# RookieJunChen/FullSubNet-plus

Hardware: AMD Instinct MI355X
Metric: STFT frames/sec (257-bin, 2 s clips), FullSubNet+ forward (higher is better)
Workload: dtype f32

## Files before the change

fullsubnet_plus_amd/_lib.py:

```python
import ctypes
import os

from . import _build

c_i32, c_i64, c_f32p, c_vp = ctypes.c_int32, ctypes.c_int64, ctypes.POINTER(ctypes.c_float), ctypes.c_void_p


class FsnpConfig(ctypes.Structure):
    _fields_ = [
        ("num_freqs", c_i32), ("look_ahead", c_i32), ("sb_num_neighbors", c_i32), ("fb_num_neighbors", c_i32),
        ("tcn_hidden", c_i32), ("num_tcn_blocks", c_i32), ("sb_hidden", c_i32), ("output_size", c_i32),
        ("norm_type", c_i32), ("fb_act", c_i32), ("sb_act", c_i32), ("kersize", c_i32 * 3),
        ("num_groups_in_drop_band", c_i32), ("attention", c_i32), ("model", c_i32), ("sequence_model", c_i32),
        ("subband_num", c_i32),
    ]


NORM_TYPES = {"offline_laplace_norm": 0, "cumulative_laplace_norm": 1, "offline_gaussian_norm": 2,
              "cumulative_layer_norm": 3}
ACTIVATIONS = {None: 0, False: 0, "": 0, "ReLU": 1, "ReLU6": 2, "Tanh": 3}
ATTENTION = {"TSSE": 0, "SE": 1, "ECA": 2, "CBAM": 3}
SEQUENCE_MODELS = {"LSTM": 0, "GRU": 1, "TCN": 2}
MODE_FULL, MODE_PARITY = 0, 1
NUM_COSTS = 27
# ... 31 lines not shown
    "fsnp_get_costs": (c_i32, [c_vp, ctypes.POINTER(ctypes.c_double * NUM_COSTS), ctypes.POINTER(c_i32), ctypes.POINTER(c_i32)]),
    "fsnp_debug_plan_rows": (c_i32, [c_i32, c_i32, c_i32, c_i32, c_i32, ctypes.c_double, ctypes.POINTER(c_i32), c_i32]),
    "fsnp_measure_costs": (c_i32, [c_vp, ctypes.POINTER(ctypes.c_double * NUM_COSTS)]),
    "fsnp_debug_set_costs": (c_i32, [c_vp, ctypes.POINTER(ctypes.c_double), c_i32]),
    "fsnp_debug_plan_rows2": (c_i32, [c_i32, c_i32, c_i32, c_i32, c_i32, ctypes.c_double, c_i32, ctypes.POINTER(ctypes.c_double),
                              ctypes.POINTER(c_i32), c_i32]),
    "fsnp_debug_coop_side_by_side": (c_i32, [ctypes.POINTER(c_i32 * 8), c_i32, c_i32, ctypes.POINTER(c_i32 * 8), c_i32, c_i32, c_i32]),
    "fsnp_debug_fullsubnet_pairing": (c_i32, [c_i32, c_i32, c_i32, ctypes.POINTER(ctypes.c_double), ctypes.POINTER(c_i32), c_i32]),
    "fsnp_debug_pipeline_pairing": (c_i32, [c_vp, c_i32, ctypes.POINTER(c_i32), c_i32]),
    "fsnp_debug_coop_chain_stats": (c_i32, [c_vp, ctypes.POINTER(c_i64 * 2), c_i32]),
    "fsnp_debug_fullband_launch": (c_i32, [c_vp, c_i32, ctypes.POINTER(c_i32 * 4)]),
    "fsnp_forward_flops": (ctypes.c_double, [c_vp, c_i32, c_i32, c_i32]),
    "fsnp_lstm_flops": (ctypes.c_double, [c_vp, c_i64, c_i32]),
    "fsnp_debug_lstm_profile": (c_i32, [c_vp, c_vp, c_vp, c_i32, c_i32, c_vp, c_i64]),
    "fsnp_debug_pp_profile": (c_i32, [c_vp, c_vp, c_vp, c_i32, c_i32, c_i32, c_vp, c_i64]),
    "fsnp_set_precision": (c_i32, [c_vp, c_i32]),
    "fsnp_check_errors": (c_i32, [c_vp]),
    "fsnp_poll_errors": (c_i32, [c_vp]),
    "fsnp_set_pipeline": (c_i32, [c_vp, c_i32]),
    "fsnp_flush": (c_i32, [c_vp, c_vp]),
    "fsnp_watch_weights": (c_i32, [c_vp, ctypes.POINTER(c_vp), ctypes.POINTER(c_i64), c_i32, c_i32, c_vp]),
    "fsnp_set_verify": (c_i32, [c_vp, c_i32]),
    "fsnp_set_verify_sample": (c_i32, [c_vp, c_i32]),
    "fsnp_verify_count": (c_i64, [c_vp]),
    "fsnp_debug_verify_sample_stats": (c_i32, [c_vp, ctypes.POINTER(c_i64 * 3)]),
    "fsnp_debug_corrupt_exchange": (c_i32, [c_vp, c_i32]),
    "fsnp_abi_version": (c_i32, []),
    "fsnp_config_size": (c_i32, []),
    "fsnp_debug_set_lstm_coop": (c_i32, [c_vp, c_i32]),
    "fsnp_debug_set_gemm_dma": (c_i32, [c_vp, c_i32]),
    "fsnp_debug_inject_error": (c_i32, [c_vp]),
    "fsnp_debug_set_chaos": (c_i32, [c_vp, c_i32]),
    "fsnp_debug_set_lstm_waves": (c_i32, [c_vp, c_i32]),
    "fsnp_debug_set_num_cus": (c_i32, [c_vp, c_i32]),
    "fsnp_debug_lstm_pack": (c_i32, [c_i32, c_i32, c_i32, c_i32, c_vp, c_vp, c_vp, c_vp, c_vp, c_i64]),
    "fsnp_debug_lstm_coop_pack": (c_i32, [c_i32, c_i32, c_i32, c_i32, c_vp, c_vp, c_vp, c_vp, c_vp, c_i64]),
    "fsnp_debug_lstm_coopw_pack": (c_i32, [c_i32, c_i32, c_i32, c_vp, c_vp, c_vp, c_vp, c_vp, c_i64]),
    "fsnp_debug_lstm_hpw_pack": (c_i32, [c_i32, c_i32, c_i32, c_vp, c_vp, c_vp, c_vp, c_vp, c_i64]),
    "fsnp_debug_lstm_fbv_pack": (c_i32, [c_i32, c_i32, c_vp, c_vp, c_vp, c_vp, c_vp, c_i64]),
    "fsnp_debug_box_probe": (c_i32, [ctypes.c_double, ctypes.POINTER(ctypes.c_double * BOX_PROBE_VALUES), c_vp]),
    "fsnp_debug_launch_clock": (c_i32, [c_vp, ctypes.POINTER(ctypes.c_double * 7)]),
    "fsnp_last_error": (ctypes.c_char_p, []),
    "fsnp_version": (ctypes.c_char_p, []),
}

LENGTHS_SYMBOLS = {
    "fsnp_forward_lengths": (c_i32, [c_vp, c_vp, c_vp, c_vp, ctypes.POINTER(c_i64 * 3 * 3), ctypes.POINTER(c_i32), c_vp, c_i32, c_i32,
                                     c_vp]),
    "fsnp_forward_complex_lengths": (c_i32, [c_vp, c_vp, ctypes.POINTER(c_i64 * 3), ctypes.POINTER(c_i32), c_vp, c_i32, c_i32, c_vp]),
    "fsnp_enhance_wave_lengths": (c_i32, [c_vp, c_vp, c_i64, c_vp, c_i64, ctypes.POINTER(c_i32), c_i32, c_i32, c_vp]),
    "fsnp_apply_cirm_lengths": (c_i32, [c_vp, c_vp, ctypes.POINTER(c_i64 * 3), c_vp, ctypes.POINTER(c_i64 * 3), ctypes.POINTER(c_i32),
                                        c_i32, c_i32, c_i32, c_vp]),
}

STREAM_SYMBOLS = {
    "fsnp_stream_create": (c_i32, [c_vp, c_i32, c_i32, ctypes.POINTER(c_vp)]),
    "fsnp_stream_destroy": (None, [c_vp]),
    "fsnp_stream_push": (c_i32, [c_vp, c_vp, ctypes.POINTER(c_i64 * 3), ctypes.POINTER(c_i32), c_vp, c_i32, c_vp]),
    "fsnp_stream_reset": (c_i32, [c_vp, ctypes.POINTER(c_i32), c_i32, c_vp]),
    "fsnp_stream_state_bytes": (c_i64, [c_vp]),
    "fsnp_stream_get_state": (c_i32, [c_vp, c_i32, c_vp, c_vp]),
    "fsnp_stream_set_state": (c_i32, [c_vp, c_i32, c_vp, c_vp]),
    "fsnp_stream_frames": (c_i32, [c_vp, c_i32, ctypes.POINTER(c_i64)]),
}

ABI_VERSION = 13
# ... 46 lines not shown
```

fullsubnet_plus_amd/csrc/fsnp_common.h:

```cpp
#pragma once
#include <hip/hip_runtime.h>
#include <math.h>
#include <stdint.h>

#include "../../include/fsnp.h"
#include "../../include/fsnp_debug.h"

namespace fsnp {

struct Dims {
    int B;
    int T;
    int Tp;
    int F;
    int FP;
    int CH;
    int H;
    int NSB;
    int NIN;
    int LA;
    const int* lens = nullptr;
    const int* tpb = nullptr;
};

// ... 135 lines not shown
struct RowDesc { int b, f, out_off, valid; };
constexpr int kGnStride = 16;

void launch_subband_stats(const Dims& d, int norm_type, const SubbandBuffers& buf, const RowDesc* rows,
                          int num_slots, hipStream_t s);
struct SbGatherArgs {
    const float* att_mag; int fb_rel, fb_branch_stride;
    const RowDesc* rows; const NormMD* md_utt; const NormMD* md_row;
    float* x; int xstride;
    int num_slots, Tp, FP, F, NSBN, NFBN, NIN;
};
void launch_sb_gather(const SbGatherArgs& a, hipStream_t s);
void launch_sb_scatter(const float* y, int ystride, const RowDesc* rows, float* out, long out_stride_o, int num_slots,
                       int Tp, int LA, int out_channels, hipStream_t s);

struct LstmWeights {
    const float* wpack;
    const float* wpack12;
    const float* wpack_bf[2];
    int ih_bf16;
    const float* wpack_coop[4];
    const float* wpack_coopn;
    const float* wpack16;
    const float* wpack16_bf;
    const float* wpack_gru;
    const float* wpack_hp;
    const float* wpack_hpw;
    int hp_wave;
    const float* wpack_fbv;
    const float* wpack_coopw;
    const float* wgen;
    int gru;
    int waves;
    const float* bias;
    const float* wfc;
    const float* bfc;
    int H, NIN, KX, OUT;
};
struct LstmArgs {
    const float* att_mag;
    const float* fb;
    int fb_rel;
    int fb_branch_stride;
    const RowDesc* rows;
    const NormMD* md_utt;
    const NormMD* md_row;
    const float* dense;
    int dense_stride;
    const NormMD* md_seq;
    float* seq_out;
    int seq_stride;
    float* out;
    long out_stride_o;
    int num_rows;
    int num_tiles;
    int ex;
    int Tp, LA, FP, F, NSBN;
    int NFBN;
    int act;
    unsigned long long* prof;
    float* coop_hx;
    unsigned* coop_bar;
    unsigned* coop_bar2;
    int coop_skew;
    unsigned* coop_err;
    unsigned* coop_abort;
    int coop_units;
    int coop_bar_stride;
    int coop_xcd;
    int coop_own_cu;
    int coop_groups;
    int coop_rows_per_group;
    int coop_corrupt;
    int coop_chaos;
    unsigned long long* clk;
    float* st_sb;
    float* st_fb;
    long st_stride;
};

struct LstmPlan { int num_tiles, ex, rows_per_slot_tile; };
LstmPlan plan_lstm_tiles(int num_rows, int num_cus);
void launch_lstm(const LstmWeights& w, const LstmArgs& a, hipStream_t s);
void launch_lstm_stream(const LstmWeights& w, const LstmArgs& a, hipStream_t s);
bool lstm_stream_available(const LstmWeights& w);
void launch_lstm16(const LstmWeights& w, const LstmArgs& a, hipStream_t s);
size_t lstm16_pack_floats(int H, int KX);
size_t lstm16_pack_floats_bf16ih(int H, int KX);
void lstm16_pack_weights_bf16ih(int H, int NIN, int KX, const float* wih0, const float* whh0, const float* wih1, const float* whh1, float* wpack);
void lstm16_pack_weights(int H, int NIN, int KX, const float* wih0, const float* whh0, const float* wih1, const float* whh1, float* wpack);
void launch_gru(const LstmWeights& w, const LstmArgs& a, hipStream_t s);
size_t gru_pack_floats(int H, int KX, int NW);
void gru_pack_weights(int H, int NIN, int KX, int NW, const float* wih0, const float* whh0, const float* wih1,
                      const float* whh1, float* wpack);
void launch_lstm_coop(const LstmWeights& w, const LstmArgs& a, hipStream_t s);
void launch_lstm_coop_seq(const LstmWeights& w, const LstmArgs& a, hipStream_t s);
size_t lstm_coop_pack_floats(int H, int KX, int units);
void lstm_coop_pack_weights(int H, int NIN, int KX, int units, const float* wih0, const float* whh0, const float* wih1,
                            const float* whh1, float* wpack);
size_t lstm_coop_exchange_bytes(int H, int row_tiles);
void launch_lstm_hp(const LstmWeights& w, const LstmArgs& a, hipStream_t s);
bool lstm_hp_available(const LstmWeights& w);
void launch_lstm_hpw(const LstmWeights& w, const LstmArgs& a, hipStream_t s);
bool lstm_hpw_available(const LstmWeights& w);
size_t lstm_hpw_pack_floats(int H, int KX);
void lstm_hpw_pack_weights(int H, int NIN, int KX, const float* wih0, const float* whh0, const float* wih1, const float* whh1, float* out);
size_t lstm_hp_pack_floats(int H, int KX);
void lstm_hp_pack_weights(int H, int NIN, int KX, const float* wih0, const float* whh0, const float* wih1, const float* whh1, float* out);
// ... 73 lines not shown
```

fullsubnet_plus_amd/csrc/fsnp_debug_abi.hip:

```cpp
#include <algorithm>
#include <string>

#include "fsnp_common.h"
#include "lstm_common.h"
#include "planner.h"
#include "fsnp_handle.h"

static double lstm_flops_per_step(const fsnp_handle* h) {
    if (h->sb_tcn) return 8 * (2.0 * h->NIN * h->CH + 2.0 * h->CH * 3 + 2.0 * h->CH * h->NIN) + 2.0 * h->NIN * h->cfg.output_size;
    const double H = h->H, NIN = h->NIN, OUT = h->cfg.output_size, G = h->NG;
    return 2.0 * G * H * (NIN + H) + 2.0 * G * H * (2 * H) + 2.0 * H * OUT;
}
static double tcn_flops_per_frame(const fsnp_handle* h) {
    const double F = h->F, CH = h->CH;
    return h->NB * (2.0 * F * CH + 2.0 * CH * 3 + 2.0 * CH * F) + 2.0 * F * F;
}
static double fb_lstm_flops_per_frame(const fsnp_handle* h) {
    const double F = h->F, CH = h->CH;
    return 2.0 * h->NG * CH * (F + CH) + 2.0 * h->NG * CH * (2 * CH) + 2.0 * CH * F;
}

extern "C" {

int fsnp_read_stage(fsnp_handle* h, const char* name, float* host_out, int64_t numel) {
// ... 275 lines not shown
    return 0;
}

int fsnp_debug_set_chaos(fsnp_handle* h, int32_t seed) {
    if (!h) { set_error("null handle"); return 1; }
    h->coop_chaos = seed;
    return 0;
}

int fsnp_debug_set_gemm_dma(fsnp_handle* h, int32_t mode) {
    if (!h || mode < 0 || mode > 3) { set_error("fsnp_debug_set_gemm_dma: mode must be 0 (general GEMM kernel), 1 (DMA kernels where they apply), 2 (as 1, never the small-batch split-K kernel) or 3 (the 128-row DMA kernel only)"); return 1; }
    h->tw.gemm_dma = mode;
    return 0;
}

int fsnp_debug_set_lstm_coop(fsnp_handle* h, int32_t mode) {
    if (!h || mode < 0 || mode > 4 || mode == 3) { set_error("fsnp_debug_set_lstm_coop: mode must be 0 (off), 1 (auto), 2 (auto, serial K-split schedule, no half-tile ping-pong kernel) or 4 (auto + the half-tile ping-pong kernel even where FSNP_COOP_HP=0)"); return 1; }
    h->planner.lstm_coop = mode != 0;
    h->coop_skew = mode != 2;
    h->planner.coop_hp = mode == 4 ? 1 : mode == 1 ? h->coop_hp_cfg : 0;
    h->fb_valu = mode == 1 || mode == 4;
    h->planner.cost.calibrated = h->calibrate ? 0 : h->planner.cost.calibrated;
    if (!h->planner.cost.calibrated) h->planner.cost = initial_costs(h->H, h->gru != 0, h->sb_tcn != 0);
    return 0;
}

int fsnp_debug_set_lstm_waves(fsnp_handle* h, int32_t waves) {
    if (!h || (waves != 0 && waves != 4 && waves != 12)) { set_error("fsnp_debug_set_lstm_waves: waves must be 0 (auto), 4 or 12"); return 1; }
    h->lstm_waves = waves;
    h->lw.waves = waves;
    return 0;
}

int fsnp_debug_set_num_cus(fsnp_handle* h, int32_t num_cus) {
    if (!h || num_cus <= 0) { set_error("fsnp_debug_set_num_cus: bad argument"); return 1; }
    h->num_cus = num_cus;
    h->tw.num_cus = num_cus;
    return 0;
}

int fsnp_debug_lstm_pack(int32_t hidden, int32_t input_size, int32_t kx, int32_t waves, const float* wih0, const float* whh0,
                         const float* wih1, const float* whh1, float* out, int64_t out_floats) {
    if (!wih0 || !whh0 || !wih1 || !whh1 || !out) { set_error("fsnp_debug_lstm_pack: null argument"); return 1; }
    if (waves <= 0 || hidden % (32 * waves) != 0 || kx % 8 != 0 || input_size > kx) { set_error("fsnp_debug_lstm_pack: bad sizes"); return 2; }
    if ((int64_t)lstm_pack_floats(hidden, kx, waves) != out_floats) {
        set_error("fsnp_debug_lstm_pack: need %lld floats", (long long)lstm_pack_floats(hidden, kx, waves));
        return 2;
    }
    lstm_pack_weights(hidden, input_size, kx, waves, wih0, whh0, wih1, whh1, out);
    return 0;
}

int fsnp_debug_lstm_coop_pack(int32_t hidden, int32_t input_size, int32_t kx, int32_t units, const float* wih0, const float* whh0,
                              const float* wih1, const float* whh1, float* out, int64_t out_floats) {
    if (!wih0 || !whh0 || !wih1 || !whh1 || !out) { set_error("fsnp_debug_lstm_coop_pack: null argument"); return 1; }
    if ((units != 8 && units != 16 && units != 32 && units != 64) || hidden % 64 != 0 || kx % 8 != 0 || input_size > kx) {
        set_error("fsnp_debug_lstm_coop_pack: bad sizes");
        return 2;
    }
    if ((int64_t)lstm_coop_pack_floats(hidden, kx, units) != out_floats) {
        set_error("fsnp_debug_lstm_coop_pack: need %lld floats", (long long)lstm_coop_pack_floats(hidden, kx, units));
        return 2;
    }
    lstm_coop_pack_weights(hidden, input_size, kx, units, wih0, whh0, wih1, whh1, out);
    return 0;
}
// ... 51 lines not shown
```

fullsubnet_plus_amd/csrc/lstm.hip:

```cpp
#include <cstring>

#include "fsnp_common.h"
#include "lstm_common.h"

namespace fsnp {

template <int EX>
__host__ __device__ __forceinline__ int e_frag_index(int e, int k) {
    return ((((k >> 3) * 2) + (k & 1)) * EX + e) * 4 + ((k >> 1) & 3);
}

struct WStream {
    __amdgpu_buffer_rsrc_t rsrc;
    int voff;
};
template <int NT>
__device__ __forceinline__ float4 wload(const WStream& ws, int g, int n) {
    const auto v = __builtin_amdgcn_raw_buffer_load_b128(ws.rsrc, ws.voff, (g * NT + n) * 1024, 0);
    return __builtin_bit_cast(float4, v);
}

template <int NT, int EX>
__device__ __forceinline__ void mfma_groups(f32x16 (&acc)[NT], float (&accx)[EX > 0 ? EX : 1][NT], float4 (&b)[NT],
                                            const float4* __restrict__ A, const float4* __restrict__ AE, int ngroups,
                                            const WStream& ws, int& gnext, int groups_total) {
    float4 a = A[0];
    float4 ae[EX > 0 ? EX : 1];
#pragma unroll
    for (int e = 0; e < EX; ++e) ae[e] = AE[e];
    for (int g = 0; g < ngroups; ++g) {
        const int gn = (g + 1 < ngroups ? g + 1 : g);
        const float4 an = A[gn * 64];
        float4 aen[EX > 0 ? EX : 1];
#pragma unroll
        for (int e = 0; e < EX; ++e) aen[e] = AE[gn * 2 * EX + e];
        if constexpr (EX == 0) {
#pragma unroll
            for (int n = 0; n < NT; ++n) {
                acc[n] = __builtin_amdgcn_mfma_f32_32x32x2f32(a.x, b[n].x, acc[n], 0, 0, 0);
                acc[n] = __builtin_amdgcn_mfma_f32_32x32x2f32(a.y, b[n].y, acc[n], 0, 0, 0);
                acc[n] = __builtin_amdgcn_mfma_f32_32x32x2f32(a.z, b[n].z, acc[n], 0, 0, 0);
                acc[n] = __builtin_amdgcn_mfma_f32_32x32x2f32(a.w, b[n].w, acc[n], 0, 0, 0);
                b[n] = wload<NT>(ws, gnext, n);
                __builtin_amdgcn_sched_barrier(0);
            }
        } else {
            constexpr int HALF = NT / 2;
#pragma unroll
            for (int hb = 0; hb < NT; hb += HALF) {
#pragma unroll
                for (int n = hb; n < hb + HALF; ++n) {
                    acc[n] = __builtin_amdgcn_mfma_f32_32x32x2f32(a.x, b[n].x, acc[n], 0, 0, 0);
                    acc[n] = __builtin_amdgcn_mfma_f32_32x32x2f32(a.y, b[n].y, acc[n], 0, 0, 0);
                    acc[n] = __builtin_amdgcn_mfma_f32_32x32x2f32(a.z, b[n].z, acc[n], 0, 0, 0);
                    acc[n] = __builtin_amdgcn_mfma_f32_32x32x2f32(a.w, b[n].w, acc[n], 0, 0, 0);
                }
                __builtin_amdgcn_sched_barrier(0);
#pragma unroll
                for (int n = hb; n < hb + HALF; ++n)
#pragma unroll
                    for (int e = 0; e < EX; ++e) {
                        float v = accx[e][n];
                        v = fmaf(ae[e].x, b[n].x, v);
                        v = fmaf(ae[e].y, b[n].y, v);
                        v = fmaf(ae[e].z, b[n].z, v);
                        accx[e][n] = fmaf(ae[e].w, b[n].w, v);
                    }
                __builtin_amdgcn_sched_barrier(0);
#pragma unroll
                for (int n = hb; n < hb + HALF; ++n) b[n] = wload<NT>(ws, gnext, n);
                __builtin_amdgcn_sched_barrier(0);
            }
        }
        gnext = (gnext + 1 == groups_total) ? 0 : gnext + 1;
        a = an;
#pragma unroll
        for (int e = 0; e < EX; ++e) ae[e] = aen[e];
    }
}

__device__ __forceinline__ unsigned short bf16_bits(float v) {
    const unsigned u = __float_as_uint(v);
    return (unsigned short)((u + 0x7FFFu + ((u >> 16) & 1u)) >> 16);
}
__host__ __device__ __forceinline__ int a_frag_index_bf16(int row, int k) {
    return (((k >> 4) * 64) + (((k >> 3) & 1) * 32) + row) * 8 + (k & 7);
}

template <int ST, int UW, int HBLO = 0>
__device__ __forceinline__ void lstm_cell(f32x16 (&acc)[4 * ST], f32x2 (&c)[ST][8], float* __restrict__ Hs, int wave,
                                          int lane, unsigned short* __restrict__ Hb = nullptr) {
#pragma unroll
    for (int s = 0; s < ST; ++s) {
        const int k = wave * UW + s * 32 + (lane & 31);
        const int kbase = (((k >> 3) * 64) + ((k & 1) * 32)) * 4 + ((k >> 1) & 3);
#pragma unroll
        for (int r = 0; r < 16; r += 2) {
            auto rd = [](float v) {
                if constexpr (ST > 1) { float o; asm("v_accvgpr_read_b32 %0, %1" : "=v"(o) : "a"(v)); return o; }
                else return v;
            };
            const f32x2 h = lstm_cell_pair(f32x2{rd(acc[s][r]), rd(acc[s][r + 1])}, f32x2{rd(acc[ST + s][r]), rd(acc[ST + s][r + 1])},
                                           f32x2{rd(acc[2 * ST + s][r]), rd(acc[2 * ST + s][r + 1])},
                                           f32x2{rd(acc[3 * ST + s][r]), rd(acc[3 * ST + s][r + 1])}, c[s][r >> 1]);
            const int row = (r & 3) + 8 * (r >> 2) + 4 * (lane >> 5);
            Hs[kbase + row * 4] = h.x;
            Hs[kbase + (row + 1) * 4] = h.y;
            if (Hb) {
                const unsigned short hx = bf16_bits(h.x), hy = bf16_bits(h.y);
                Hb[a_frag_index_bf16(row, k)] = hx; Hb[a_frag_index_bf16(row + 1, k)] = hy;
                if constexpr (HBLO > 0) {
// ... 175 lines not shown
    float* Xf = reinterpret_cast<float*>(Xs);
    float* XEf = reinterpret_cast<float*>(XEs);
    {
        const NormMD m0 = md_row ? md_row[0] : md;
#pragma unroll
        for (int i = 0; i < NG; ++i)
            if (goff[i] != -2) Xf[xdst[i]] = goff[i] >= 0 ? (gbase[goff[i]] - m0.m) / m0.d : 0.0f;
        if (havex) {
            const NormMD mx = mdx_row ? mdx_row[0] : mdx;
            XEf[xdstx] = goffx >= 0 ? (gbase[goffx] - mx.m) / mx.d : 0.0f;
        }
    }

    const float* __restrict__ bias_l0 = BF ? nullptr : Bs + ((0 * NW + wave) * NT) * 32 + (lane & 31);
    const float* __restrict__ bias_l1 = Bs + (((BL - 1) * NW + wave) * NT) * 32 + (lane & 31);
    f32x2 c0[ST][8], c1[ST][8];
    float cx0[EXA][ST], cx1[EXA][ST];
#pragma unroll
    for (int s = 0; s < ST; ++s) {
#pragma unroll
        for (int r = 0; r < 8; ++r) { c0[s][r] = f32x2{0.0f, 0.0f}; c1[s][r] = f32x2{0.0f, 0.0f}; }
#pragma unroll
        for (int e = 0; e < EXA; ++e) { cx0[e][s] = 0.0f; cx1[e][s] = 0.0f; }
    }

    WStream ws;
    ws.rsrc = __builtin_amdgcn_make_buffer_rsrc(const_cast<float*>(w.wpack) + (size_t)wave * KGT * NT * 256, 0,
                                                KGT * NT * 1024, 0x00020000);
    ws.voff = lane * 16;
    float4 breg[NT];
#pragma unroll
    for (int n = 0; n < NT; ++n) breg[n] = wload<NT>(ws, 0, n);
    int gnext = 1;
    auto run_groups = [&](f32x16 (&acc_)[NT], float (&accx_)[EXA][NT], const float4* A_, const float4* AE_, int ng) {
        mfma_groups<NT, EX>(acc_, accx_, breg, A_, AE_, ng, ws, gnext, KGT);
    };

    const int fc_row = (wave & 3) * 8 + (lane & 7);
    const int fc_o = (lane >> 3) & 1;
    const int fc_kp = lane >> 4;
    const RowDesc fc_rd = rows_s[fc_row];
    const RowDesc fcx_rd = (EX > 0 && wave < EX) ? rows_s[32 + (wave < EX ? wave : 0)] : RowDesc{0, 0, 0, 0};

    auto fc_store = [&](int t_of_h) {
      if (wave < 4) {
        constexpr int KGP = KGH / 4;
        float sum = 0.0f;
#pragma unroll 4
        for (int kk = 0; kk < KGP; ++kk) {
            const int kg = fc_kp * KGP + kk;
#pragma unroll
            for (int kh = 0; kh < 2; ++kh) {
                const float4 h4 = H1s[kg * 64 + kh * 32 + fc_row];
                const float4 w4 = Wfc4[(fc_o * KGH + kg) * 2 + kh];
                sum += h4.x * w4.x + h4.y * w4.y + h4.z * w4.z + h4.w * w4.w;
            }
        }
        sum += __shfl_xor(sum, 16);
        sum += __shfl_xor(sum, 32);
        if (fc_kp == 0 && fc_rd.valid && t_of_h >= a.LA)
            a.out[(size_t)fc_rd.out_off + (size_t)fc_o * a.out_stride_o + (t_of_h - a.LA)] = apply_act(sum + w.bfc[fc_o], a.act);
      }
        if (EX > 0 && wave < EX) {
            const int o = lane >> 5;
            const float* he = reinterpret_cast<const float*>(HE1s);
            float sx = 0.0f;
#pragma unroll 4
            for (int i = 0; i < HID / 32; ++i) {
                const int k = (lane & 31) + 32 * i;
                sx += he[e_frag_index<EXA>(wave, k)] * w.wfc[o * HID + k];
            }
#pragma unroll
            for (int m = 16; m > 0; m >>= 1) sx += __shfl_xor(sx, m);
            if ((lane & 31) == 0 && fcx_rd.valid && t_of_h >= a.LA)
                a.out[(size_t)fcx_rd.out_off + (size_t)o * a.out_stride_o + (t_of_h - a.LA)] = apply_act(sx + w.bfc[o], a.act);
        }
    };

    const float4* AEx = XEs + (lane >> 5) * EX;
    const float4* AEh0 = HE0s + (lane >> 5) * EX;
    const float4* AEh1 = HE1s + (lane >> 5) * EX;

    __syncthreads();

    unsigned long long* prof = nullptr;
    int prof_stride = 0;
    if constexpr (PROF) {
        const bool rec = blockIdx.x == 0 && tid == 0;
        prof = a.prof + (rec ? 0 : (size_t)Tp * 8 + (size_t)blockIdx.x * 256 + tid);
        prof_stride = rec ? 8 : 0;
    }
#define FSNP_STAMP(i) do { if constexpr (PROF) prof[t * prof_stride + (prof_stride ? (i) : 0)] = __builtin_amdgcn_s_memtime(); } while (0)

    for (int t = 0; t < Tp; ++t) {
        FSNP_STAMP(0);
        float xr[NG], xrx = 0.0f;
        NormMD mdn = md, mdxn = mdx;
        const bool have_next = (t + 1 < Tp);
        if (have_next) {
            if (md_row) mdn = md_row[t + 1];
#pragma unroll
            for (int i = 0; i < NG; ++i) xr[i] = goff[i] >= 0 ? gbase[goff[i] + (t + 1) * gstep] : 0.0f;
            if (havex) {
                if (mdx_row) mdxn = mdx_row[t + 1];
                xrx = goffx >= 0 ? gbase[goffx + (t + 1) * gstep] : 0.0f;
            }
        }

        f32x16 acc[NT];
        float accx[EXA][NT];
#pragma unroll
        for (int n = 0; n < NT; ++n) {
#pragma unroll
            for (int r = 0; r < 16; ++r) acc[n][r] = BF ? 0.0f : bias_l0[n * 32];
#pragma unroll
            for (int e = 0; e < EXA; ++e) accx[e][n] = 0.0f;
        }
        run_groups(acc, accx, Xs + lane, AEx, KG0);
        FSNP_STAMP(1);
        __syncthreads();
        FSNP_STAMP(2);
        lstm_cell<ST, UW, HILO ? KSB * 64 * 8 : 0>(acc, c0, reinterpret_cast<float*>(H0s), wave, lane, BF ? reinterpret_cast<unsigned short*>(H0b) : nullptr);
        if (EX > 0) lstm_cell_extra<ST, UW, EX, NT>(accx, cx0, bias_l0, reinterpret_cast<float*>(HE0s), wave, lane);
        if (have_next) {
#pragma unroll
            for (int i = 0; i < NG; ++i)
                if (goff[i] != -2) Xf[xdst[i]] = goff[i] >= 0 ? (xr[i] - mdn.m) / mdn.d : 0.0f;
            if (havex) XEf[xdstx] = goffx >= 0 ? (xrx - mdxn.m) / mdxn.d : 0.0f;
        }
        if (t > 0) fc_store(t - 1);
        FSNP_STAMP(3);
        __syncthreads();
        FSNP_STAMP(4);
#pragma unroll
        for (int n = 0; n < NT; ++n) {
#pragma unroll
            for (int r = 0; r < 16; ++r) acc[n][r] = bias_l1[n * 32];
#pragma unroll
            for (int e = 0; e < EXA; ++e) accx[e][n] = 0.0f;
        }
        run_groups(acc, accx, H1s + lane, AEh1, KGH);
        if constexpr (BF) mfma_groups_bf16<NT, EX, HILO ? KSB * 64 : 0>(acc, accx, breg, H0b + lane, HE0s, KSB, ws, gnext, KGT, lane);
        else run_groups(acc, accx, H0s + lane, AEh0, KGH);
        FSNP_STAMP(5);
        __syncthreads();
        FSNP_STAMP(6);
        lstm_cell<ST, UW>(acc, c1, reinterpret_cast<float*>(H1s), wave, lane);
        if (EX > 0) lstm_cell_extra<ST, UW, EX, NT>(accx, cx1, bias_l1, reinterpret_cast<float*>(HE1s), wave, lane);
        FSNP_STAMP(7);
    }
#undef FSNP_STAMP
    __syncthreads();
    fc_store(Tp - 1);
    if (a.clk != nullptr && tid == 0) {
        const unsigned long long m1 = __builtin_amdgcn_s_memtime(), r1 = __builtin_amdgcn_s_memrealtime();
        if (blockIdx.x == 0) { a.clk[2] = m1; a.clk[3] = r1; }
        atomicMax(a.clk + 4, r1 - clk_s[1]);
        atomicMax(a.clk + 5, m1 - clk_s[0]);
        atomicMin(a.clk + 6, r1 - clk_s[1]);
    }
}

size_t lstm_pack_floats(int H, int KX, int NW) {
    const int NT = 4 * (H / NW / 32);
    const int KGT = KX / 8 + H / 8 + 2 * (H / 8);
    return (size_t)NW * KGT * NT * 64 * 4;
}

void lstm_pack_weights(int H, int NIN, int KX, int NW, const float* wih0, const float* whh0, const float* wih1,
                       const float* whh1, float* wpack) {
    const int UW = H / NW, ST = UW / 32, NT = 4 * ST;
    const int KGX = KX / 8, KGH = H / 8, KG0 = KGX + KGH, KGT = KG0 + 2 * KGH;
    for (int wv = 0; wv < NW; ++wv)
        for (int g = 0; g < KGT; ++g)
            for (int n = 0; n < NT; ++n)
                for (int lane = 0; lane < 64; ++lane)
// ... 29 lines not shown
void lstm_pack_weights_bf16ih(int H, int NIN, int KX, int NW, const float* wih0, const float* whh0, const float* wih1,
                              const float* whh1, const float* bias0, float* wpack) {
    const int UW = H / NW, ST = UW / 32, NT = 4 * ST;
    const int KGX = KX / 8, KGH = H / 8, KG0 = KGX + KGH, KSB = H / 16, KGT = KG0 + KGH + KSB;
    for (int wv = 0; wv < NW; ++wv)
        for (int g = 0; g < KGT; ++g)
            for (int n = 0; n < NT; ++n)
                for (int lane = 0; lane < 64; ++lane) {
                    const int gate = n / ST, s = n % ST;
                    const int wrow = gate * H + wv * UW + s * 32 + (lane & 31);
                    float* dst = wpack + ((((size_t)wv * KGT + g) * NT + n) * 64 + lane) * 4;
                    if (g < KG0 + KGH) {
                        for (int p = 0; p < 4; ++p) {
                            float v = 0.0f;
                            if (g < KG0) {
                                const int k = 8 * g + 2 * p + (lane >> 5);
                                if (k < KX) { if (k < NIN) v = wih0[(size_t)wrow * NIN + k]; else if (k == NIN) v = bias0[wrow]; }
                                else v = whh0[(size_t)wrow * H + (k - KX)];
                            } else {
                                const int k = 8 * (g - KG0) + 2 * p + (lane >> 5);
                                v = whh1[(size_t)wrow * H + k];
                            }
                            dst[p] = v;
                        }
                    } else {
                        const int ks = g - KG0 - KGH;
                        unsigned short* d16 = reinterpret_cast<unsigned short*>(dst);
                        for (int j = 0; j < 8; ++j) d16[j] = host_bf16(wih1[(size_t)wrow * H + 16 * ks + 8 * (lane >> 5) + j]);
                    }
                }
}

template <int EX, int NW, bool BF, int KX, int HID = 384>
static void launch_lstm_ex(const LstmWeights& w, const LstmArgs& a, hipStream_t s) {
    constexpr int OUT = 2;
    constexpr int KGX = KX / 8, KGH = HID / 8, NT = 4 * (HID / NW / 32);
    const size_t smem = (size_t)(KGX + 2 * KGH) * (64 + 2 * EX) * 16 + (size_t)OUT * KGH * 2 * 16 +
                        (32 + EX) * sizeof(RowDesc) + (size_t)(BF ? 1 : 2) * NW * NT * 32 * 4 + (BF ? (size_t)(EX == 0 ? 2 : 1) * (HID / 16) * 64 * 16 : 0);
    LstmWeights wv = w;
    wv.wpack = BF ? (NW == 12 ? w.wpack_bf[1] : w.wpack_bf[0]) : (NW == 12 ? w.wpack12 : w.wpack);
    if constexpr (KX == 40 && HID == 384) {
        if (a.prof != nullptr) {
            auto kern = lstm2_fc_kernel<HID, KX, OUT, EX, true, NW, BF>;
            (void)hipFuncSetAttribute(reinterpret_cast<const void*>(kern), hipFuncAttributeMaxDynamicSharedMemorySize, (int)smem);
            hipLaunchKernelGGL(kern, dim3(a.num_tiles), dim3(64 * NW), smem, s, wv, a);
            return;
        }
    }
    auto kern = lstm2_fc_kernel<HID, KX, OUT, EX, false, NW, BF>;
    static PerDeviceOnce attr_once;
    attr_once.run([&] { (void)hipFuncSetAttribute(reinterpret_cast<const void*>(kern), hipFuncAttributeMaxDynamicSharedMemorySize, (int)smem); });
    hipLaunchKernelGGL(kern, dim3(a.num_tiles), dim3(64 * NW), smem, s, wv, a);
}

template <int NW, bool BF, int KX>
static void launch_lstm_nw(const LstmWeights& w, const LstmArgs& a, hipStream_t s) {
    switch (a.ex) {
        case 0: launch_lstm_ex<0, NW, BF, KX>(w, a, s); break;
        case 1: launch_lstm_ex<1, NW, BF, KX>(w, a, s); break;
        case 2: launch_lstm_ex<2, NW, BF, KX>(w, a, s); break;
        default: launch_lstm_ex<4, NW, BF, KX>(w, a, s); break;
    }
}

void launch_lstm(const LstmWeights& w, const LstmArgs& a, hipStream_t s) {
    if (a.num_tiles <= 0) return;
    const int waves = w.waves != 0 ? w.waves : (a.ex > 0 ? 12 : 4);
    if (w.H == 256) {
        if (w.KX == 64) launch_lstm_ex<0, 4, false, 64, 256>(w, a, s);
        else launch_lstm_ex<0, 4, false, 40, 256>(w, a, s);
        return;
    }
    if (w.KX == 64) {
// ... 91 lines not shown
    {
        const RowDesc rd = rows_s[grow];
#pragma unroll
        for (int i = 0; i < NG; ++i) {
            const int j = (tid >> 5) + JSTEP * i;
            goff[i] = j >= KX ? -2 : (rd.valid > 0 && j < w.NIN)
                          ? sb_feature_offset(j, rd.f, rd.b * Tp * a.FP, a.F, a.NSBN, a.NFBN, a.fb_rel, a.fb_branch_stride) : -1;
            xdst[i] = a_frag_index(grow, j < KX ? j : 0);
        }
        md_row = a.md_row + (size_t)(slot0 + grow) * Tp;
    }
    float* Xf = reinterpret_cast<float*>(Xs);
    {
        const NormMD m0 = rows_s[grow].valid > 0 ? md_row[0] : NormMD{0.0f, 1.0f};
#pragma unroll
        for (int i = 0; i < NG; ++i)
            if (goff[i] != -2) Xf[xdst[i]] = goff[i] >= 0 ? (gbase[goff[i]] - m0.m) / m0.d : 0.0f;
    }

    const float* __restrict__ bias_l0 = Bs + ((0 * NW + wave) * NT) * 32 + (lane & 31);
    const float* __restrict__ bias_l1 = Bs + ((1 * NW + wave) * NT) * 32 + (lane & 31);
    f32x2 c0[ST][8], c1[ST][8];
    stream_state_io<ST, UW, HID, true>(c0, c1, reinterpret_cast<float*>(H0s), reinterpret_cast<float*>(H1s), rows_s, a.st_sb, a.st_stride, 0,
                                       wave, lane);

    WStream ws;
    ws.rsrc = __builtin_amdgcn_make_buffer_rsrc(const_cast<float*>(w.wpack) + (size_t)wave * KGT * NT * 256, 0, KGT * NT * 1024, 0x00020000);
    ws.voff = lane * 16;
    float4 breg[NT];
#pragma unroll
    for (int n = 0; n < NT; ++n) breg[n] = wload<NT>(ws, 0, n);
    int gnext = 1;
    float accx[1][NT];
    auto run_groups = [&](f32x16 (&acc_)[NT], const float4* A_, int ng) {
        mfma_groups<NT, 0>(acc_, accx, breg, A_, A_, ng, ws, gnext, KGT);
    };

    const int fc_row = (wave & 3) * 8 + (lane & 7);
    const int fc_o = (lane >> 3) & 1;
    const int fc_kp = lane >> 4;
    const RowDesc fc_rd = rows_s[fc_row];
    auto fc_store = [&](int t_of_h) {
        constexpr int KGP = KGH / 4;
        float sum = 0.0f;
#pragma unroll 4
        for (int kk = 0; kk < KGP; ++kk) {
            const int kg = fc_kp * KGP + kk;
#pragma unroll
            for (int kh = 0; kh < 2; ++kh) {
                const float4 h4 = H1s[kg * 64 + kh * 32 + fc_row];
                const float4 w4 = Wfc4[(fc_o * KGH + kg) * 2 + kh];
                sum += h4.x * w4.x + h4.y * w4.y + h4.z * w4.z + h4.w * w4.w;
            }
        }
        sum += __shfl_xor(sum, 16);
        sum += __shfl_xor(sum, 32);
        if (fc_kp == 0 && t_of_h < fc_rd.valid)
            a.out[(size_t)fc_rd.out_off + (size_t)fc_o * a.out_stride_o + t_of_h] = apply_act(sum + w.bfc[fc_o], a.act);
    };

    __syncthreads();

    for (int t = 0; t < nsteps; ++t) {
        float xr[NG];
        NormMD mdn = {0.0f, 1.0f};
        const bool have_next = (t + 1 < nsteps);
        if (have_next) {
            if (rows_s[grow].valid > 0) mdn = md_row[t + 1];
#pragma unroll
            for (int i = 0; i < NG; ++i) xr[i] = goff[i] >= 0 ? gbase[goff[i] + (t + 1) * gstep] : 0.0f;
        }

        f32x16 acc[NT];
#pragma unroll
        for (int n = 0; n < NT; ++n)
#pragma unroll
            for (int r = 0; r < 16; ++r) acc[n][r] = bias_l0[n * 32];
        run_groups(acc, Xs + lane, KG0);
        __syncthreads();
        lstm_cell<ST, UW>(acc, c0, reinterpret_cast<float*>(H0s), wave, lane);
        if (have_next) {
#pragma unroll
            for (int i = 0; i < NG; ++i)
                if (goff[i] != -2) Xf[xdst[i]] = goff[i] >= 0 ? (xr[i] - mdn.m) / mdn.d : 0.0f;
        }
        if (t > 0) fc_store(t - 1);
        __syncthreads();
#pragma unroll
        for (int n = 0; n < NT; ++n)
#pragma unroll
            for (int r = 0; r < 16; ++r) acc[n][r] = bias_l1[n * 32];
        run_groups(acc, H1s + lane, KGH);
        run_groups(acc, H0s + lane, KGH);
        __syncthreads();
        lstm_cell<ST, UW>(acc, c1, reinterpret_cast<float*>(H1s), wave, lane);
        if (t + 1 == nsteps || mixed)
            stream_state_io<ST, UW, HID, false>(c0, c1, reinterpret_cast<float*>(H0s), reinterpret_cast<float*>(H1s), rows_s, a.st_sb,
                                                a.st_stride, t + 1, wave, lane);
    }
    __syncthreads();
    fc_store(nsteps - 1);
}

template <int HID, int KX>
static void launch_lstm_stream_one(const LstmWeights& w, const LstmArgs& a, hipStream_t s) {
    constexpr int KGX = KX / 8, KGH = HID / 8, NT = 4 * (HID / 4 / 32);
    const size_t smem = (size_t)(KGX + 2 * KGH) * 64 * 16 + (size_t)2 * KGH * 2 * 16 + 32 * sizeof(RowDesc) + (size_t)2 * 4 * NT * 32 * 4;
    auto kern = lstm2_fc_stream_kernel<HID, KX>;
    static PerDeviceOnce attr_once;
    attr_once.run([&] { (void)hipFuncSetAttribute(reinterpret_cast<const void*>(kern), hipFuncAttributeMaxDynamicSharedMemorySize, (int)smem); });
    hipLaunchKernelGGL(kern, dim3(a.num_tiles), dim3(256), smem, s, w, a);
}

bool lstm_stream_available(const LstmWeights& w) {
    return !w.gru && w.OUT == 2 && (w.H == 384 || w.H == 256) && (w.KX == 40 || w.KX == 64) && w.wpack != nullptr;
}

void launch_lstm_stream(const LstmWeights& w, const LstmArgs& a, hipStream_t s) {
    if (a.num_tiles <= 0) return;
    if (w.H == 256) { if (w.KX == 64) launch_lstm_stream_one<256, 64>(w, a, s); else launch_lstm_stream_one<256, 40>(w, a, s); }
    else if (w.KX == 64) launch_lstm_stream_one<384, 64>(w, a, s);
    else launch_lstm_stream_one<384, 40>(w, a, s);
}

LstmPlan plan_lstm_tiles(int num_rows, int num_cus) {
    LstmPlan p{};
// ... 17 lines not shown
```

fullsubnet_plus_amd/model.py:

```python
import ctypes
import operator
import weakref

import torch
import torch.nn as nn

from . import _lib

_TCN_DILATIONS = (1, 2, 5, 9, 1, 2, 5, 9)

_TREE_GENERATION = [0]


def _bump_tree_generation(*_args, **_kwargs):
    _TREE_GENERATION[0] += 1


nn.modules.module.register_module_parameter_registration_hook(_bump_tree_generation)
nn.modules.module.register_module_module_registration_hook(_bump_tree_generation)


class _StageHolder(nn.Module):

    def __getstate__(self):
# ... 569 lines not shown
        with torch.cuda.device(noisy_complex.device):
            if lengths is not None:
                _lib.check(_lib.load().fsnp_apply_cirm_lengths(mask.data_ptr(), xr.data_ptr(), ctypes.byref(st), orr.data_ptr(),
                                                               ctypes.byref(ost), lengths, B, F, T, ctypes.c_void_p(stream)),
                           "fsnp_apply_cirm_lengths")
            else:
                _lib.check(_lib.load().fsnp_apply_cirm(mask.data_ptr(), xr.data_ptr(), ctypes.byref(st), orr.data_ptr(),
                                                       ctypes.byref(ost), B, F, T, ctypes.c_void_p(stream)), "fsnp_apply_cirm")
        return out

    def lstm2_fc(self, x):
        assert x.dim() == 3 and x.is_cuda
        lib = self._ensure_handle(x.device)
        n, _, steps = x.shape
        xt = x.permute(0, 2, 1).contiguous().float()
        out = torch.empty((n, self.output_size, steps), dtype=torch.float32, device=x.device)
        stream = torch.cuda.current_stream(x.device).cuda_stream
        with torch.cuda.device(x.device):
            _lib.check(lib.fsnp_lstm2_fc(self._handle, xt.data_ptr(), out.data_ptr(), n, steps,
                                         ctypes.c_void_p(stream)), "fsnp_lstm2_fc")
        return out

    def read_stage(self, name, batch, frames):
        lib = _lib.load()
        rows = batch if name.startswith("gate_") else batch * (frames + self.look_ahead)
        host = torch.empty((rows, self.num_freqs), dtype=torch.float32)
        _lib.check(lib.fsnp_read_stage(self._handle, name.encode(), host.data_ptr(), host.numel()), "fsnp_read_stage")
        return host if name.startswith("gate_") else host.view(batch, frames + self.look_ahead, self.num_freqs)

    def debug_set_num_cus(self, num_cus, device="cuda"):
        lib = self._ensure_handle(_resolve_device(device))
        _lib.check(lib.fsnp_debug_set_num_cus(self._handle, int(num_cus)), "fsnp_debug_set_num_cus")

    def debug_set_lstm_waves(self, waves, device="cuda"):
        lib = self._ensure_handle(_resolve_device(device))
        _lib.check(lib.fsnp_debug_set_lstm_waves(self._handle, int(waves)), "fsnp_debug_set_lstm_waves")

    def debug_set_lstm_coop(self, mode, device="cuda"):
        lib = self._ensure_handle(_resolve_device(device))
        _lib.check(lib.fsnp_debug_set_lstm_coop(self._handle, int(mode)), "fsnp_debug_set_lstm_coop")
        self.__dict__["_lstm_coop_mode"] = int(mode)

    def debug_set_gemm_dma(self, mode, device="cuda"):
        lib = self._ensure_handle(_resolve_device(device))
        _lib.check(lib.fsnp_debug_set_gemm_dma(self._handle, int(mode)), "fsnp_debug_set_gemm_dma")

    def set_precision(self, mode, device="cuda"):
        assert mode in ("fp32", "bf16_ih")
        lib = self._ensure_handle(_resolve_device(device))
        _lib.check(lib.fsnp_set_precision(self._handle, {"fp32": 0, "bf16_ih": 1}[mode]), "fsnp_set_precision")

    def debug_set_chaos(self, seed, device="cuda"):
        lib = self._ensure_handle(_resolve_device(device))
        _lib.check(lib.fsnp_debug_set_chaos(self._handle, int(seed)), "fsnp_debug_set_chaos")

    def debug_inject_error(self):
        _lib.check(_lib.load().fsnp_debug_inject_error(self._handle), "fsnp_debug_inject_error")

    def check_errors(self):
        _lib.check(_lib.load().fsnp_check_errors(self._handle), "fsnp_check_errors")

    def set_timing(self, enable=True):
        _lib.check(_lib.load().fsnp_set_timing(self._handle, int(bool(enable))), "fsnp_set_timing")

    def get_timing(self, reset=True):
        ms = (ctypes.c_double * 4)()
# ... 284 lines not shown
```

include/fsnp_debug.h:

```cpp
#ifndef FSNP_DEBUG_H
#define FSNP_DEBUG_H

#include "fsnp.h"

#ifdef __cplusplus
extern "C" {
#endif

int fsnp_read_stage(fsnp_handle* h, const char* name, float* host_out, int64_t numel);

int fsnp_set_timing(fsnp_handle* h, int32_t enable);
int fsnp_get_timing(fsnp_handle* h, double ms[4], int64_t count[4], int32_t reset);
int fsnp_describe_plan(const fsnp_handle* h, int32_t batch, int32_t mode, int32_t* out, int32_t max_chunks);
int fsnp_describe_plan_ex(const fsnp_handle* h, int32_t batch, int32_t mode, int32_t* out, int32_t max_chunks);
#define FSNP_NUM_COSTS 27
int fsnp_get_costs(const fsnp_handle* h, double out[FSNP_NUM_COSTS], int32_t* calibrated, int32_t* occ);
int fsnp_measure_costs(fsnp_handle* h, double out[FSNP_NUM_COSTS]);
int fsnp_debug_plan_rows(int32_t num_rows, int32_t num_cus, int32_t hidden, int32_t gru, int32_t coop, double composite_gain,
                         int32_t* out, int32_t max_chunks);

int fsnp_debug_coop_side_by_side(const int32_t a_per_xcd[8], int32_t a_own_cu, int32_t a_per_cu, const int32_t b_per_xcd[8],
                                 int32_t b_own_cu, int32_t b_per_cu, int32_t cus_per_xcd);
int fsnp_debug_fullsubnet_pairing(int32_t batch, int32_t num_cus, int32_t fb_workgroups_per_cu, const double* costs, int32_t* out,
                                  int32_t max_records);
int fsnp_debug_pipeline_pairing(const fsnp_handle* h, int32_t batch, int32_t* out, int32_t max_records);
int fsnp_debug_coop_chain_stats(fsnp_handle* h, int64_t out[2], int32_t reset);
int fsnp_debug_fullband_launch(const fsnp_handle* h, int32_t batch, int32_t out[4]);

int fsnp_debug_set_costs(fsnp_handle* h, const double* costs, int32_t workgroups_per_cu);
int fsnp_debug_plan_rows2(int32_t num_rows, int32_t num_cus, int32_t hidden, int32_t gru, int32_t coop, double composite_gain,
                          int32_t workgroups_per_cu, const double* costs, int32_t* out, int32_t max_chunks);

double fsnp_forward_flops(const fsnp_handle* h, int32_t batch, int32_t frames, int32_t mode);
double fsnp_lstm_flops(const fsnp_handle* h, int64_t num_seq, int32_t steps);

int fsnp_debug_pp_profile(fsnp_handle* h, const float* x, float* out, int32_t num_seq, int32_t steps, int32_t tiles_per_group,
                          uint64_t* host_stamps, int64_t num_stamps);
int fsnp_debug_lstm_profile(fsnp_handle* h, const float* x, float* out, int32_t num_seq, int32_t steps,
                            uint64_t* host_stamps, int64_t num_stamps);
int fsnp_debug_corrupt_exchange(fsnp_handle* h, int32_t step);

int fsnp_debug_set_lstm_coop(fsnp_handle* h, int32_t mode);
int fsnp_debug_set_gemm_dma(fsnp_handle* h, int32_t mode);
int fsnp_debug_inject_error(fsnp_handle* h);

int fsnp_debug_set_chaos(fsnp_handle* h, int32_t seed);

int fsnp_debug_set_lstm_waves(fsnp_handle* h, int32_t waves);

int fsnp_debug_set_num_cus(fsnp_handle* h, int32_t num_cus);

int fsnp_debug_lstm_pack(int32_t hidden, int32_t input_size, int32_t kx, int32_t waves, const float* wih0, const float* whh0,
                         const float* wih1, const float* whh1, float* out, int64_t out_floats);
int fsnp_debug_lstm_coop_pack(int32_t hidden, int32_t input_size, int32_t kx, int32_t units, const float* wih0,
                              const float* whh0, const float* wih1, const float* whh1, float* out, int64_t out_floats);

int fsnp_debug_lstm_coopw_pack(int32_t hidden, int32_t input_size, int32_t kx, const float* wih0, const float* whh0, const float* wih1,
                               const float* whh1, float* out, int64_t out_floats);

int fsnp_debug_lstm_hpw_pack(int32_t hidden, int32_t input_size, int32_t kx, const float* wih0, const float* whh0, const float* wih1,
                             const float* whh1, float* out, int64_t out_floats);

int fsnp_debug_lstm_fbv_pack(int32_t hidden, int32_t input_size, const float* wih0, const float* whh0, const float* wih1, const float* whh1,
                             float* out, int64_t out_floats);

int fsnp_debug_verify_sample_stats(const fsnp_handle* h, int64_t out[3]);

#define FSNP_BOX_PROBE_VALUES 9
int fsnp_debug_box_probe(double target_ms, double out[FSNP_BOX_PROBE_VALUES], void* hip_stream);
#define FSNP_LAUNCH_CLOCK_VALUES 7
int fsnp_debug_launch_clock(fsnp_handle* h, double out[FSNP_LAUNCH_CLOCK_VALUES]);

#ifdef __cplusplus
}
#endif
#endif
```

Measured before the change: 143,900.

## Skip zero-padded input pairs and zero initial hidden state in LSTM MFMA loop

The fused LSTM kernel now stops the input-projection MFMA chain at the last live input pair rather than running over the full padded KX width. At t=0 it also skips the recurrent-weight groups because the hidden state is still zero. The weight-stream cursor is now passed explicitly as a 'gafter' group index so the prefetched weight registers stay aligned when groups are skipped. The FC store exits early for look-ahead frames, and a debug toggle restores the old full-work path. This adds branching inside an unrolled MFMA schedule, and the weight-prefetch bookkeeping risks misalignment with the packed stream.

Measured after the change: 144,300 (median of 6 runs). Within noise of the previous version (+0.3%).

```diff
diff --git a/fullsubnet_plus_amd/_lib.py b/fullsubnet_plus_amd/_lib.py
--- a/fullsubnet_plus_amd/_lib.py
+++ b/fullsubnet_plus_amd/_lib.py
@@ -87,6 +87,7 @@
     "fsnp_debug_inject_error": (c_i32, [c_vp]),
     "fsnp_debug_set_chaos": (c_i32, [c_vp, c_i32]),
     "fsnp_debug_set_lstm_waves": (c_i32, [c_vp, c_i32]),
+    "fsnp_debug_set_zero_skip": (c_i32, [c_vp, c_i32]),
     "fsnp_debug_set_num_cus": (c_i32, [c_vp, c_i32]),
     "fsnp_debug_lstm_pack": (c_i32, [c_i32, c_i32, c_i32, c_i32, c_vp, c_vp, c_vp, c_vp, c_vp, c_i64]),
     "fsnp_debug_lstm_coop_pack": (c_i32, [c_i32, c_i32, c_i32, c_i32, c_vp, c_vp, c_vp, c_vp, c_vp, c_i64]),
diff --git a/fullsubnet_plus_amd/csrc/fsnp_common.h b/fullsubnet_plus_amd/csrc/fsnp_common.h
--- a/fullsubnet_plus_amd/csrc/fsnp_common.h
+++ b/fullsubnet_plus_amd/csrc/fsnp_common.h
@@ -191,6 +191,7 @@
     const float* wgen;
     int gru;
     int waves;
+    int no_zero_skip;
     const float* bias;
     const float* wfc;
     const float* bfc;
@@ -233,6 +234,7 @@
     int coop_corrupt;
     int coop_chaos;
     unsigned long long* clk;
+    int x_pairs, skip0;
     float* st_sb;
     float* st_fb;
     long st_stride;
diff --git a/fullsubnet_plus_amd/csrc/fsnp_debug_abi.hip b/fullsubnet_plus_amd/csrc/fsnp_debug_abi.hip
--- a/fullsubnet_plus_amd/csrc/fsnp_debug_abi.hip
+++ b/fullsubnet_plus_amd/csrc/fsnp_debug_abi.hip
@@ -331,6 +331,12 @@
     return 0;
 }
 
+int fsnp_debug_set_zero_skip(fsnp_handle* h, int32_t on) {
+    if (!h) { set_error("null handle"); return 1; }
+    h->lw.no_zero_skip = on ? 0 : 1;
+    return 0;
+}
+
 int fsnp_debug_set_num_cus(fsnp_handle* h, int32_t num_cus) {
     if (!h || num_cus <= 0) { set_error("fsnp_debug_set_num_cus: bad argument"); return 1; }
     h->num_cus = num_cus;
diff --git a/fullsubnet_plus_amd/csrc/lstm.hip b/fullsubnet_plus_amd/csrc/lstm.hip
--- a/fullsubnet_plus_amd/csrc/lstm.hip
+++ b/fullsubnet_plus_amd/csrc/lstm.hip
@@ -20,16 +20,19 @@
     return __builtin_bit_cast(float4, v);
 }
 
-template <int NT, int EX>
+template <int NT, int EX, int UNROLL = 1>
 __device__ __forceinline__ void mfma_groups(f32x16 (&acc)[NT], float (&accx)[EX > 0 ? EX : 1][NT], float4 (&b)[NT],
                                             const float4* __restrict__ A, const float4* __restrict__ AE, int ngroups,
-                                            const WStream& ws, int& gnext, int groups_total) {
+                                            const WStream& ws, int& gnext, int gafter) {
     float4 a = A[0];
     float4 ae[EX > 0 ? EX : 1];
 #pragma unroll
     for (int e = 0; e < EX; ++e) ae[e] = AE[e];
+#pragma unroll UNROLL
     for (int g = 0; g < ngroups; ++g) {
         const int gn = (g + 1 < ngroups ? g + 1 : g);
+        int gl = (g + 1 < ngroups ? gnext : gafter);
+        if constexpr (EX == 0) asm volatile("" : "+s"(gl));
         const float4 an = A[gn * 64];
         float4 aen[EX > 0 ? EX : 1];
 #pragma unroll
@@ -41,7 +44,7 @@
                 acc[n] = __builtin_amdgcn_mfma_f32_32x32x2f32(a.y, b[n].y, acc[n], 0, 0, 0);
                 acc[n] = __builtin_amdgcn_mfma_f32_32x32x2f32(a.z, b[n].z, acc[n], 0, 0, 0);
                 acc[n] = __builtin_amdgcn_mfma_f32_32x32x2f32(a.w, b[n].w, acc[n], 0, 0, 0);
-                b[n] = wload<NT>(ws, gnext, n);
+                b[n] = wload<NT>(ws, gl, n);
                 __builtin_amdgcn_sched_barrier(0);
             }
         } else {
@@ -68,15 +71,53 @@
                     }
                 __builtin_amdgcn_sched_barrier(0);
 #pragma unroll
-                for (int n = hb; n < hb + HALF; ++n) b[n] = wload<NT>(ws, gnext, n);
+                for (int n = hb; n < hb + HALF; ++n) b[n] = wload<NT>(ws, gl, n);
                 __builtin_amdgcn_sched_barrier(0);
             }
         }
-        gnext = (gnext + 1 == groups_total) ? 0 : gnext + 1;
+        gnext = gl + 1;
         a = an;
 #pragma unroll
         for (int e = 0; e < EX; ++e) ae[e] = aen[e];
     }
+}
+
+template <int NT, int EX>
+__device__ __forceinline__ void mfma_part_group(f32x16 (&acc)[NT], float (&accx)[EX > 0 ? EX : 1][NT], float4 (&b)[NT],
+                                                const float4* __restrict__ A, const float4* __restrict__ AE, int np,
+                                                const WStream& ws, int& gnext, int gafter) {
+    const float4 a0 = A[0];
+    float4 ae0[EX > 0 ? EX : 1];
+#pragma unroll
+    for (int e = 0; e < EX; ++e) ae0[e] = AE[e];
+#pragma unroll
+    for (int n = 0; n < NT; ++n) {
+        const float4 a = a0, bn = b[n];
+        const float4 (&ae)[EX > 0 ? EX : 1] = ae0;
+        if (np > 0) {
+        acc[n] = __builtin_amdgcn_mfma_f32_32x32x2f32(a.x, bn.x, acc[n], 0, 0, 0);
+#pragma unroll
+        for (int e = 0; e < EX; ++e) accx[e][n] = fmaf(ae[e].x, bn.x, accx[e][n]);
+        if (np > 1) {
+            acc[n] = __builtin_amdgcn_mfma_f32_32x32x2f32(a.y, bn.y, acc[n], 0, 0, 0);
+#pragma unroll
+            for (int e = 0; e < EX; ++e) accx[e][n] = fmaf(ae[e].y, bn.y, accx[e][n]);
+            if (np > 2) {
+                acc[n] = __builtin_amdgcn_mfma_f32_32x32x2f32(a.z, bn.z, acc[n], 0, 0, 0);
+#pragma unroll
+                for (int e = 0; e < EX; ++e) accx[e][n] = fmaf(ae[e].z, bn.z, accx[e][n]);
+                if (np > 3) {
+                    acc[n] = __builtin_amdgcn_mfma_f32_32x32x2f32(a.w, bn.w, acc[n], 0, 0, 0);
+#pragma unroll
+                    for (int e = 0; e < EX; ++e) accx[e][n] = fmaf(ae[e].w, bn.w, accx[e][n]);
+                }
+            }
+        }
+        }
+        b[n] = wload<NT>(ws, gafter, n);
+        __builtin_amdgcn_sched_barrier(0);
+    }
+    gnext = gafter + 1;
 }
 
 __device__ __forceinline__ unsigned short bf16_bits(float v) {
@@ -318,9 +359,10 @@
 #pragma unroll
     for (int n = 0; n < NT; ++n) breg[n] = wload<NT>(ws, 0, n);
     int gnext = 1;
-    auto run_groups = [&](f32x16 (&acc_)[NT], float (&accx_)[EXA][NT], const float4* A_, const float4* AE_, int ng) {
-        mfma_groups<NT, EX>(acc_, accx_, breg, A_, AE_, ng, ws, gnext, KGT);
+    auto run_groups = [&](f32x16 (&acc_)[NT], float (&accx_)[EXA][NT], const float4* A_, const float4* AE_, int ng, int gafter) {
+        mfma_groups<NT, EX>(acc_, accx_, breg, A_, AE_, ng, ws, gnext, gafter);
     };
+    const int nxp = a.x_pairs - 4 * (KGX - 1);
 
     const int fc_row = (wave & 3) * 8 + (lane & 7);
     const int fc_o = (lane >> 3) & 1;
@@ -329,6 +371,7 @@
     const RowDesc fcx_rd = (EX > 0 && wave < EX) ? rows_s[32 + (wave < EX ? wave : 0)] : RowDesc{0, 0, 0, 0};
 
     auto fc_store = [&](int t_of_h) {
+      if (t_of_h < a.LA) return;
       if (wave < 4) {
         constexpr int KGP = KGH / 4;
         float sum = 0.0f;
@@ -344,7 +387,7 @@
         }
         sum += __shfl_xor(sum, 16);
         sum += __shfl_xor(sum, 32);
-        if (fc_kp == 0 && fc_rd.valid && t_of_h >= a.LA)
+        if (fc_kp == 0 && fc_rd.valid)
             a.out[(size_t)fc_rd.out_off + (size_t)fc_o * a.out_stride_o + (t_of_h - a.LA)] = apply_act(sum + w.bfc[fc_o], a.act);
       }
         if (EX > 0 && wave < EX) {
@@ -358,7 +401,7 @@
             }
 #pragma unroll
             for (int m = 16; m > 0; m >>= 1) sx += __shfl_xor(sx, m);
-            if ((lane & 31) == 0 && fcx_rd.valid && t_of_h >= a.LA)
+            if ((lane & 31) == 0 && fcx_rd.valid)
                 a.out[(size_t)fcx_rd.out_off + (size_t)o * a.out_stride_o + (t_of_h - a.LA)] = apply_act(sx + w.bfc[o], a.act);
         }
     };
@@ -402,7 +445,14 @@
 #pragma unroll
             for (int e = 0; e < EXA; ++e) accx[e][n] = 0.0f;
         }
-        run_groups(acc, accx, Xs + lane, AEx, KG0);
+        const bool skip_h = EX == 0 && a.skip0 != 0 && t == 0;
+        if constexpr (EX == 0) {
+            mfma_groups<NT, EX, KGX - 1>(acc, accx, breg, Xs + lane, AEx, KGX - 1, ws, gnext, KGX - 1);
+            mfma_part_group<NT, EX>(acc, accx, breg, Xs + (KGX - 1) * 64 + lane, AEx + (KGX - 1) * 2 * EX, nxp, ws, gnext, KGX);
+            run_groups(acc, accx, H0s + lane, AEh0, skip_h ? 1 : KGH, KG0);
+        } else {
+            run_groups(acc, accx, Xs + lane, AEx, KG0, KG0);
+        }
         FSNP_STAMP(1);
         __syncthreads();
         FSNP_STAMP(2);
@@ -425,9 +475,9 @@
 #pragma unroll
             for (int e = 0; e < EXA; ++e) accx[e][n] = 0.0f;
         }
-        run_groups(acc, accx, H1s + lane, AEh1, KGH);
+        run_groups(acc, accx, H1s + lane, AEh1, skip_h ? 1 : KGH, KG0 + KGH);
         if constexpr (BF) mfma_groups_bf16<NT, EX, HILO ? KSB * 64 : 0>(acc, accx, breg, H0b + lane, HE0s, KSB, ws, gnext, KGT, lane);
-        else run_groups(acc, accx, H0s + lane, AEh0, KGH);
+        else run_groups(acc, accx, H0s + lane, AEh0, KGH, 0);
         FSNP_STAMP(5);
         __syncthreads();
         FSNP_STAMP(6);
@@ -523,13 +573,17 @@
 }
 
 template <int EX, int NW, bool BF, int KX, int HID = 384>
-static void launch_lstm_ex(const LstmWeights& w, const LstmArgs& a, hipStream_t s) {
+static void launch_lstm_ex(const LstmWeights& w, const LstmArgs& a_in, hipStream_t s) {
     constexpr int OUT = 2;
     constexpr int KGX = KX / 8, KGH = HID / 8, NT = 4 * (HID / NW / 32);
     const size_t smem = (size_t)(KGX + 2 * KGH) * (64 + 2 * EX) * 16 + (size_t)OUT * KGH * 2 * 16 +
                         (32 + EX) * sizeof(RowDesc) + (size_t)(BF ? 1 : 2) * NW * NT * 32 * 4 + (BF ? (size_t)(EX == 0 ? 2 : 1) * (HID / 16) * 64 * 16 : 0);
     LstmWeights wv = w;
     wv.wpack = BF ? (NW == 12 ? w.wpack_bf[1] : w.wpack_bf[0]) : (NW == 12 ? w.wpack12 : w.wpack);
+    LstmArgs a = a_in;
+    const int live = (w.NIN + (BF ? 1 : 0) + 1) / 2;
+    a.x_pairs = w.no_zero_skip || live > KX / 2 ? KX / 2 : live < 4 * (KGX - 1) ? 4 * (KGX - 1) : live;
+    a.skip0 = w.no_zero_skip ? 0 : 1;
     if constexpr (KX == 40 && HID == 384) {
         if (a.prof != nullptr) {
             auto kern = lstm2_fc_kernel<HID, KX, OUT, EX, true, NW, BF>;
@@ -687,8 +741,8 @@
     for (int n = 0; n < NT; ++n) breg[n] = wload<NT>(ws, 0, n);
     int gnext = 1;
     float accx[1][NT];
-    auto run_groups = [&](f32x16 (&acc_)[NT], const float4* A_, int ng) {
-        mfma_groups<NT, 0>(acc_, accx, breg, A_, A_, ng, ws, gnext, KGT);
+    auto run_groups = [&](f32x16 (&acc_)[NT], const float4* A_, int ng, int gafter) {
+        mfma_groups<NT, 0>(acc_, accx, breg, A_, A_, ng, ws, gnext, gafter);
     };
 
     const int fc_row = (wave & 3) * 8 + (lane & 7);
@@ -731,7 +785,7 @@
         for (int n = 0; n < NT; ++n)
 #pragma unroll
             for (int r = 0; r < 16; ++r) acc[n][r] = bias_l0[n * 32];
-        run_groups(acc, Xs + lane, KG0);
+        run_groups(acc, Xs + lane, KG0, KG0);
         __syncthreads();
         lstm_cell<ST, UW>(acc, c0, reinterpret_cast<float*>(H0s), wave, lane);
         if (have_next) {
@@ -745,8 +799,8 @@
         for (int n = 0; n < NT; ++n)
 #pragma unroll
             for (int r = 0; r < 16; ++r) acc[n][r] = bias_l1[n * 32];
-        run_groups(acc, H1s + lane, KGH);
-        run_groups(acc, H0s + lane, KGH);
+        run_groups(acc, H1s + lane, KGH, KG0 + KGH);
+        run_groups(acc, H0s + lane, KGH, 0);
         __syncthreads();
         lstm_cell<ST, UW>(acc, c1, reinterpret_cast<float*>(H1s), wave, lane);
         if (t + 1 == nsteps || mixed)
diff --git a/fullsubnet_plus_amd/model.py b/fullsubnet_plus_amd/model.py
--- a/fullsubnet_plus_amd/model.py
+++ b/fullsubnet_plus_amd/model.py
@@ -625,6 +625,10 @@
         lib = self._ensure_handle(_resolve_device(device))
         _lib.check(lib.fsnp_debug_set_num_cus(self._handle, int(num_cus)), "fsnp_debug_set_num_cus")
 
+    def debug_set_zero_skip(self, on, device="cuda"):
+        lib = self._ensure_handle(_resolve_device(device))
+        _lib.check(lib.fsnp_debug_set_zero_skip(self._handle, 1 if on else 0), "fsnp_debug_set_zero_skip")
+
     def debug_set_lstm_waves(self, waves, device="cuda"):
         lib = self._ensure_handle(_resolve_device(device))
         _lib.check(lib.fsnp_debug_set_lstm_waves(self._handle, int(waves)), "fsnp_debug_set_lstm_waves")
diff --git a/include/fsnp_debug.h b/include/fsnp_debug.h
--- a/include/fsnp_debug.h
+++ b/include/fsnp_debug.h
@@ -48,6 +48,8 @@
 
 int fsnp_debug_set_lstm_waves(fsnp_handle* h, int32_t waves);
 
+int fsnp_debug_set_zero_skip(fsnp_handle* h, int32_t on);
+
 int fsnp_debug_set_num_cus(fsnp_handle* h, int32_t num_cus);
 
 int fsnp_debug_lstm_pack(int32_t hidden, int32_t input_size, int32_t kx, int32_t waves, const float* wih0, const float* whh0,
```
